# SCoulY/MuSCLe

Hardware: AMD Instinct MI355X
Metric: images/sec (whole node), MCL EfficientNet-B7 448x448 bs=32/GPU (higher is better)
Workload: dtype f32; 1 GPU; train_mcl.py loop body, step-A (epoch-4 gates: focal+softmargin+pairwise+ER+IMC, one backward, one Adam step), MuSCLe(efficientnet-b7, last_pooling=False, 21 classes), random-init weights; per_gpu_batch=32, global_batch=32, image=448x448, parallelism=single, optimizer=Adam(lr=1e-4, wd=5e-5) fused, launch=eager, weight-gradient GEMMs on a second stream

## Files before the change

include/muscle_hip.h:

```cpp
#ifndef MUSCLE_HIP_H
#define MUSCLE_HIP_H

#ifdef __cplusplus
extern "C" {
#endif

int mx_version(void);
int mx_abi_hash(void);
const char* mx_last_error(void);


int mx_pw_fwd_parts(int M, int N, int K);
int mx_pw_fwd(const float* A, int a_mode, const float* a_scale, const float* a_shift, const float* a_gate,
              int rows_per_sample, const float* W, float* C, int M, int K, int N, int lda, int ldc,
              const float* bias, const float* residual, int relu, float* stats, void* stream);

int mx_set_gemm_mode(int mode);
int mx_get_gemm_mode(void);
int mx_set_wgrad_kernel(int kernel, int groups);
int mx_get_wgrad_kernel(void);
int mx_gemm_uses_split(int kind, int M, int N, int K);

long mx_pw_planes_bytes(int N, int K);
int mx_pw_planes_tiles(int N, int K);
int mx_pw_planes_batch(const long* table, int n, int total_tiles, void* stream);
int mx_pw_fwd_uses_planes(int M, int K, int N);
int mx_pw_fwd_planes(const float* A, const void* Wplanes, float* C, int M, int K, int N, int lda, int ldc,
                     const float* bias, const float* residual, int relu, float* stats, void* stream);

int mx_transpose(const float* src, float* dst, int rows, int cols, void* stream);
int mx_transpose_batch(const long* table, int n, int total_tiles, void* stream);

int mx_pw_dgrad(const float* G, const float* W, float* dX, int M, int K, int N, int ldg, int ldx,
                const float* residual, void* stream);

int mx_pw_dgrad_bnbwd(const float* G, const float* X, const float* coef, const float* Wt, float* dX, float* dZ, int M, int K, int N,
                      int ldg, int ldx, const float* residual, void* stream);

int mx_pw_fwd_act_uses_planes(int M, int K, int N);
int mx_pw_fwd_planes_act(const float* A, const float* scale, const float* shift, const float* gate, int rows_per_sample,
                         const void* Wplanes, float* C, int M, int K, int N, int lda, int ldc, float* stats, void* stream);

int mx_pw_dgrad_bnbwd_planes(const float* G, const float* X, const float* coef, const void* WtPlanes, float* dX, int M, int K, int N,
                             int ldg, int ldx, const float* residual, void* stream);
int mx_pw_wgrad_tile_bnbwd_ok(int R, int Co, int Ci);
int mx_pw_wgrad_small_bnbwd_ok(int R, int Co, int Ci);
int mx_pw_wgrad_small_bnbwd(const float* G, const float* G2, const float* coef, const float* X, float* dW, int R, int Co, int Ci,
                            int ldg, int ldx, void* ws, long ws_bytes, void* stream);
int mx_pw_wgrad_tile_bnbwd(const float* G, const float* G2, const float* coef, const float* X, float* dW, int R, int Co, int Ci,
                           int ldg, int ldx, void* ws, long ws_bytes, void* stream);
int mx_pw_wgrad_tile_bnbwd_dz_ok(int R, int Co, int Ci, int ldg, int ldx);
int mx_pw_wgrad_tile_bnbwd_dz(const float* G, const float* G2, const float* coef, const float* X, float* dW, float* dz, int R, int Co,
                              int Ci, int ldg, int ldx, void* ws, long ws_bytes, void* stream);

long mx_pw_wgrad_ws(int R, int Co, int Ci);
int mx_pw_wgrad(const float* G, const float* X, int x_mode, const float* x_scale, const float* x_shift,
                const float* x_gate, int rows_per_sample, float* dW, int R, int Co, int Ci, int ldg, int ldx,
                void* ws, long ws_bytes, void* stream);

long mx_pw_wgrad_small_ws(int R, int Co, int Ci, int x_mode);
int mx_pw_wgrad_small(const float* G, const float* X, int x_mode, const float* x_scale, const float* x_shift,
                      const float* x_gate, int rows_per_sample, float* dW, int R, int Co, int Ci, int ldg, int ldx,
                      void* ws, long ws_bytes, void* stream);

int mx_pw_bwd_small_fused_ok(int R, int Co, int Ci);
int mx_pw_bwd_small_fused_groups(int R, int Co, int Ci);
int mx_pw_bwd_small_fused(const float* G, const float* G2, const float* coef, const float* X, const float* W, float* dW, float* dX,
                          const float* residual, int R, int Co, int Ci, int ldg, int ldx, int lddx, void* ws, long ws_bytes, void* stream);
int mx_pw_parts_reduce(const float* part, int groups, int n, float* dW, void* stream);

int mx_pw_proj_bwd_fused_ok(int R, int Cout, int Cexp, int rows_per_sample);
int mx_pw_proj_bwd_fused_groups(int R, int Cout, int Cexp, int rows_per_sample);
int mx_pw_proj_bwd_fused(const float* dp, const float* d_raw, const float* scale, const float* shift, const float* gate, int rows_per_sample,
                         const float* Wp, float* dW, float* dA, float* out5, int R, int Cout, int Cexp, int lddp, int ldraw, int ldda,
                         void* ws, long ws_bytes, void* stream);

long mx_pw_wgrad_tile_ws(int R, int Co, int Ci, int x_mode);
int mx_pw_wgrad_tile(const float* G, const float* X, int x_mode, const float* x_scale, const float* x_shift,
                     const float* x_gate, int rows_per_sample, float* dW, int R, int Co, int Ci, int ldg, int ldx,
                     void* ws, long ws_bytes, void* stream);

int mx_bgemm(int layout, const float* A, const float* B, float* C, int M, int N, int K, int lda, int ldb, int ldc,
             long sa, long sb, long sc, int batch, int relu, void* stream);


int mx_colreduce_parts(long rows, int C);
int mx_colstats(const float* X, long rows, int C, float* part, void* stream);

int mx_bn_finalize(const float* part, int P, int C, double count, const float* gamma, const float* beta, float* running_mean,
                   float* running_var, float momentum, float eps, int training, float* scale, float* shift,
                   float* mean, float* rstd, double* acc , void* stream);

int mx_fold_block(const float* We, const float* g0, const float* b0, const float* m0, const float* v0, float eps0,
                  const float* g1, const float* b1, const float* m1, const float* v1, float eps1,
                  const float* Wp, const float* g2, const float* b2, const float* m2, const float* v2, float eps2,
                  int Cin, int Cexp, int Cout, float* We_f, float* be, float* s1, float* t1, float* Wp_f, float* bp, void* stream);

int mx_bn_apply(const float* P, const float* scale, const float* shift, const float* row_scale, const float* residual,
                const float* gate, float* out, long rows, int C, int rows_per_sample, int act, void* stream);

int mx_bn_bwd_reduce(const float* G, const float* X, const float* row_scale, const float* gate, const float* gate_add,
                     const float* act_scale, const float* act_shift, long rows, int C, int rows_per_sample,
                     float* part, void* stream);

int mx_bn_bwd_finalize(const float* part, int P, int C, double count, const float* gamma, const float* mean, const float* rstd,
                       int training, float* dgamma, float* dbeta, float* c1, float* c2, float* c3, double* acc,
                       void* stream);

int mx_bn_bwd_apply(const float* G, const float* X, const float* row_scale, const float* gate, const float* gate_add,
                    const float* act_scale, const float* act_shift, const float* c1, const float* c2, const float* c3,
                    float* out, long rows, int C, int rows_per_sample, void* stream);

long mx_pool_ws(long rows, int C, int rows_per_sample, int planes);
int mx_pool_sum(const float* X, const float* G, const float* scale, const float* shift, int act, long rows, int C,
                int rows_per_sample, float* out, void* ws, long ws_bytes, void* stream);

int mx_se_bn1_pool(const float* dA, const float* X, const float* scale, const float* shift, long rows, int C, int rows_per_sample,
                   float* out5, void* ws, long ws_bytes, void* stream);
int mx_bn1_sums_finalize(const float* pooled5, const float* gate, const float* gh, const float* W1, float inv_hw, float* add,
                         int N, int C, int SQ, double count, const float* gamma, const float* mean, const float* rstd, int training,
                         float* dgamma, float* dbeta, float* c1, float* c2, float* c3, void* stream);


int mx_dwconv_fwd_parts(int N, int Ho, int Wo, int C, int S);
long mx_dwconv_fwd_ws(int N, int Ho, int Wo, int C, int S);
int mx_dwconv_fwd(const float* X, const float* scale, const float* shift, const float* W, float* Y, float* stats,
                  const float* pool_scale, const float* pool_shift, float* pooled, void* ws, long ws_bytes, int N,
                  int H, int Wd, int C, int K, int S, int pad_lo, int Ho, int Wo, void* stream);

int mx_dwconv_bwd_data(const float* dY, const float* W, const float* residual, float* dX, int N, int H, int Wd, int C,
                       int K, int S, int pad_lo, int Ho, int Wo, void* stream);

int mx_dwconv_bwd_weight_parts(int N, int Ho, int Wo, int C, int S);
int mx_dwconv_bwd_weight(const float* X, const float* scale, const float* shift, const float* dY, float* dW, float* dw_scratch,
                         int N, int H, int Wd, int C, int K, int S, int pad_lo, int Ho, int Wo, void* stream);

int mx_dwconv_bwd_fused_parts(int N, int H, int Wd, int C, int K);
int mx_dwconv_bwd_fused(const float* dA, const float* D, const float* gate, const float* add, const float* a1, const float* b1,
                        const float* c1, const float* c2, const float* c3, const float* X, const float* a0, const float* b0,
                        const float* W, const float* residual, float* gX, float* dW, float* dw_scratch, float* part, int N, int H,
                        int Wd, int C, int K, int pad_lo, void* stream);

int mx_dwconv_bwd_fused_bn0(const float* dA, const float* D, const float* gate, const float* add, const float* a1, const float* b1,
                            const float* c1, const float* c2, const float* c3, const float* X, const float* a0, const float* b0,
                            const float* W, float* gX, float* dW, float* dw_scratch, float* part, int N, int H, int Wd, int C, int K,
                            int pad_lo, void* ws, long ws_bytes, double count, const float* gamma, const float* mean, const float* rstd,
                            int training, float* dgamma, float* dbeta, float* o1, float* o2, float* o3, void* stream);

int mx_dwconv_bwd_fused_s2_parts(int N, int H, int Wd, int C, int K);
int mx_dwconv_bwd_fused_s2(const float* dA, const float* D, const float* gate, const float* add, const float* a1, const float* b1,
                           const float* c1, const float* c2, const float* c3, const float* X, const float* a0, const float* b0,
                           const float* W, float* gX, float* dW, float* dw_scratch, float* part, int N, int H, int Wd, int C, int K,
                           int pad_lo, int Ho, int Wo, void* stream);

int mx_dw_parts_reduce(const float* part, int P, int n, float* dW, void* stream);


int mx_se_fwd(const float* pooled_sum, float inv_hw, const float* W1, const float* b1, const float* W2, const float* b2,
// ... 233 lines not shown
```

muscle_amd/engine.py:

```python
from __future__ import annotations

import os

from dataclasses import dataclass, field
from typing import Dict, List, Optional

import torch

from . import ops
from .arch import BlockCfg, NetCfg
from .ops import BNState


@dataclass
class BlockTape:
    cfg: BlockCfg
    H: int
    W: int
    Ho: int
    Wo: int
    x: torch.Tensor
    x_st: Optional[BNState]
    e_raw: Optional[torch.Tensor] = None
    bn0: Optional[BNState] = None
# ... 205 lines not shown
            t.x = None
            tape.blocks.append(t)
            if b.index == 0:
                tape.cols = tape.stem_raw = None
            if len(tape.blocks) >= 2 and tape.blocks[-2].cfg.index not in cfg.taps:
                tape.blocks[-2].out = None
            x, x_st, h, w = t.out, None, ho, wo
            continue
        M, Mo = N * h * w, N * ho * wo
        if b.expand:
            assert x_st is None
            st0 = None
            t.e_raw = ops.pw_fwd(x.view(M, b.cin), m._expand_conv.weight.view(b.cexp, b.cin), b.cexp, want_stats=training,
                                 planes=tape.wp.get(id(m._expand_conv.weight)))
            if training:
                t.e_raw, st0 = t.e_raw
            t.e_raw = t.e_raw.view(N, h, w, b.cexp)
            t.bn0 = ops.bn_finalize(st0, M, m._bn0, training)
            dw_in, dw_st = t.e_raw, t.bn0
        else:
            dw_in, dw_st = x, x_st
        st1 = None
        t.d_raw = ops.dwconv_fwd(dw_in, m._depthwise_conv.weight, b.kernel, b.stride, b.pad_lo, ho, wo, st=dw_st,
                                 want_stats=training)
        if training:
            t.d_raw, st1 = t.d_raw
        t.bn1 = ops.bn_finalize(st1, Mo, m._bn1, training)
        d2 = t.d_raw.view(Mo, b.cexp)
        pooled = ops.pool_sum(d2, ho * wo, st=t.bn1, act=True)
        t.s, t.h, t.gate = ops.se_fwd(pooled, 1.0 / (ho * wo), m._se_reduce.weight.view(b.se, b.cexp), m._se_reduce.bias,
                                      m._se_expand.weight.view(b.cexp, b.se), m._se_expand.bias)
        st2 = None
        if b.cout > MATERIALISE_ABOVE:
            t.a = ops.bn_apply(d2, t.bn1, gate=t.gate, rows_per_sample=ho * wo, act=True)
            t.p_raw = ops.pw_fwd(t.a, m._project_conv.weight.view(b.cout, b.cexp), b.cout, want_stats=training,
                                 planes=tape.wp.get(id(m._project_conv.weight)))
        else:
            t.p_raw = ops.pw_fwd(d2, m._project_conv.weight.view(b.cout, b.cexp), b.cout, a_mode=ops.BNACT,
                                 a_scale=t.bn1.scale, a_shift=t.bn1.shift, a_gate=t.gate, rows_per_sample=ho * wo,
                                 want_stats=training, planes=tape.wp.get(id(m._project_conv.weight)))
        if training:
            t.p_raw, st2 = t.p_raw
        t.bn2 = ops.bn_finalize(st2, Mo, m._bn2, training)
        if b.skip and training and b.drop_rate:
            if drop_u is not None:
                keep = 1.0 - b.drop_rate
                t.row_scale = torch.floor(keep + drop_u[b.index].to(dev, torch.float32)) / keep
            else:
                t.row_scale = drop_scales[b.index]
        res = None
        if b.skip:
            assert x_st is None
            res = x.view(M, b.cin)
        t.out = ops.bn_apply(t.p_raw, t.bn2, row_scale=t.row_scale, residual=res, rows_per_sample=ho * wo).view(N, ho, wo, b.cout)
        tape.blocks.append(t)
        x, x_st, h, w = t.out, None, ho, wo
        if not save:
            t.x = t.e_raw = t.d_raw = t.p_raw = t.a = None
            if b.index == 0:
                tape.cols = tape.stem_raw = None
            if len(tape.blocks) >= 2 and tape.blocks[-2].cfg.index not in cfg.taps:
                tape.blocks[-2].out = None
    ops.flush_batch_counters()
    return tape


class GradSink:

    def __init__(self):
        self.bufs: Dict[int, torch.Tensor] = {}

    def of(self, p: torch.nn.Parameter) -> torch.Tensor:
        g = self.bufs.get(id(p))
        if g is None:
            g = torch.zeros_like(p, memory_format=torch.contiguous_format)
            self.bufs[id(p)] = g
        return g


FOLD_BN0_EARLY = os.environ.get("MUSCLE_FOLD_BN0_EARLY", "1") == "1"
DW_S2_FUSED = os.environ.get("MUSCLE_DW_S2_FUSED", "1") == "1"
PW_BWD_FUSED = os.environ.get("MUSCLE_PW_BWD_FUSED", "1") == "1"
PW_PROJ_BWD_FUSED = os.environ.get("MUSCLE_PW_PROJ_BWD_FUSED", "1") == "1"
WGRAD_SIDE_STREAM = os.environ.get("MUSCLE_WGRAD_STREAM", "1") == "1"
_side_streams: Dict[int, "torch.cuda.Stream"] = {}


class _WgradLane:
    def __init__(self, device):
        self.s = None
        self.pending = []
        self.keep = []
        if WGRAD_SIDE_STREAM:
            key = device.index if device.index is not None else torch.cuda.current_device()
            if key not in _side_streams:
                _side_streams[key] = torch.cuda.Stream(device=device)
            self.s = _side_streams[key]

    def _queue(self, launch, *reads):
        if self.s is None:
            return launch()
        self.pending.append((launch, reads))

    def wgrad(self, G, X, dW, **kw):
        return self._queue(lambda: ops.pw_wgrad(G, X, dW, **kw), G, X)

    def wgrad_bnbwd(self, G, G2, coef, X, dW):
        return self._queue(lambda: ops.pw_wgrad_bnbwd(G, G2, coef, X, dW), G, X, G2, coef)

    def dw_reduce(self, scratch, dW):
        return self._queue(lambda: ops.dw_parts_reduce(scratch, dW), scratch)

    def pw_reduce(self, part, dW):
        return self._queue(lambda: ops.pw_parts_reduce(part, dW), part)

    def flush(self):
        if self.s is None or not self.pending:
            return
        self.s.wait_stream(torch.cuda.current_stream())
        with torch.cuda.stream(self.s):
            for launch, _ in self.pending:
                launch()
        self.keep.extend(reads for _, reads in self.pending)
        self.pending = []

    def progress(self, done, module):
        if self.s is None:
            return done(module)
        self.flush()
        self.s.wait_stream(torch.cuda.current_stream())
        with torch.cuda.stream(self.s):
            done(module)

    def join(self):
        self.flush()
        if self.s is not None:
            torch.cuda.current_stream().wait_stream(self.s)
        self.keep = []


def _dw_input(t: BlockTape):
    return (t.e_raw, t.bn0) if t.cfg.expand else (t.x, t.x_st)


def _project_backward(lane, tape: Tape, t: BlockTape, m, g_out, sink: GradSink):
    b, hw = t.cfg, t.Ho * t.Wo
    Mo = tape.N * hw
    dp = ops.bn_backward(g_out.reshape(Mo, b.cout), t.p_raw, m._bn2, t.bn2, sink.of(m._bn2.weight), sink.of(m._bn2.bias), tape.training,
                         row_scale=t.row_scale, rows_per_sample=hw)
    if t.a is None and PW_PROJ_BWD_FUSED:
        takes = getattr(ops, "pw_proj_bwd_fused_takes", None)
        if takes is not None and takes(Mo, b.cout, b.cexp, hw):
            ga, pooled5 = ops.pw_proj_bwd_fused(dp, t.d_raw.view(Mo, b.cexp), t.bn1, t.gate, hw, m._project_conv.weight.view(b.cout, b.cexp),
                                                sink.of(m._project_conv.weight).view(b.cout, b.cexp), defer=lane.pw_reduce)
            lane.flush()
            return ga, pooled5
    if t.a is not None:
        lane.wgrad(dp, t.a, sink.of(m._project_conv.weight).view(b.cout, b.cexp))
        t.a = None
    else:
        lane.wgrad(dp, t.d_raw.view(Mo, b.cexp), sink.of(m._project_conv.weight).view(b.cout, b.cexp), x_mode=ops.BNACT,
                   x_scale=t.bn1.scale, x_shift=t.bn1.shift, x_gate=t.gate, rows_per_sample=hw)
    ga = ops.pw_dgrad(dp, m._project_conv.weight.view(b.cout, b.cexp), b.cexp, wt=tape.wt.get(id(m._project_conv.weight)),
                      planes=tape.wtp.get(id(m._project_conv.weight)))
    lane.flush()
    return ga, None


def _se_bn1_coeffs(tape: Tape, t: BlockTape, m, ga, pooled5, sink: GradSink):
    b, hw = t.cfg, t.Ho * t.Wo
    Mo = tape.N * hw
    if pooled5 is None:
        pooled5 = ops.se_bn1_pool(ga, t.d_raw.view(Mo, b.cexp), t.bn1, hw)
    gh = ops.se_bwd(pooled5[0], t.gate, t.s, t.h, m._se_expand.weight.view(b.cexp, b.se),
                    sink.of(m._se_reduce.weight).view(b.se, b.cexp), sink.of(m._se_reduce.bias),
                    sink.of(m._se_expand.weight).view(b.cexp, b.se), sink.of(m._se_expand.bias))
    return ops.bn1_coeffs(pooled5, t.gate, gh, m._se_reduce.weight.view(b.se, b.cexp), 1.0 / hw, Mo, m._bn1, t.bn1,
                          sink.of(m._bn1.weight), sink.of(m._bn1.bias), tape.training)


def _depthwise_backward(lane, tape: Tape, t: BlockTape, m, ga, c1, add, skip_res, sink: GradSink):
    b, N = t.cfg, tape.N
    dw_in, dw_st = _dw_input(t)
    res = None if dw_st is not None else skip_res
    if b.stride == 1 and b.pad_lo == (b.kernel - 1) // 2:
        return ops.dwconv_bwd_fused(ga.view(N, t.Ho, t.Wo, b.cexp), t.d_raw, t.gate, add, t.bn1, c1, dw_in, dw_st,
                                    m._depthwise_conv.weight, sink.of(m._depthwise_conv.weight), b.kernel, b.pad_lo,
                                    residual=res, defer=lane.dw_reduce)
    if DW_S2_FUSED and b.stride == 2 and dw_st is not None:
        return ops.dwconv_bwd_fused_s2(ga.view(N, t.Ho, t.Wo, b.cexp), t.d_raw, t.gate, add, t.bn1, c1, dw_in, dw_st,
                                       m._depthwise_conv.weight, sink.of(m._depthwise_conv.weight), b.kernel, b.pad_lo,
                                       defer=lane.dw_reduce)
    dd = ops.bn_backward_from_coeffs(ga, t.d_raw.view(N * t.Ho * t.Wo, b.cexp), t.bn1, c1, gate=t.gate, gate_add=add,
                                     rows_per_sample=t.Ho * t.Wo, out=ga).view(N, t.Ho, t.Wo, b.cexp)
    ops.dwconv_bwd_weight(dw_in, dd, sink.of(m._depthwise_conv.weight), b.kernel, b.stride, b.pad_lo, st=dw_st)
    return ops.dwconv_bwd_data(dd, m._depthwise_conv.weight, b.kernel, b.stride, b.pad_lo, t.H, t.W, residual=res), None


def _bn0_expand_backward(lane, backbone, cfg: NetCfg, tape: Tape, t: BlockTape, m, gx, part0, skip_res, sink: GradSink):
    b, N, training = t.cfg, tape.N, tape.training
    dw_in, dw_st = _dw_input(t)
    bn_mod = m._bn0 if b.expand else backbone._bn0
    M = N * t.H * t.W
    raw2, gx2 = dw_in.view(M, dw_in.shape[3]), gx.view(M, dw_in.shape[3])
    res = skip_res.reshape(M, b.cin) if skip_res is not None else None
    if part0 is not None:
        c0 = ops.bn_bwd_coeffs(part0, M, bn_mod, dw_st, sink.of(bn_mod.weight), sink.of(bn_mod.bias), training)
        wtp = tape.wtp.get(id(m._expand_conv.weight)) if b.expand else None
        takes = None
        if FOLD_BN0_EARLY and b.expand and (wtp is not None if b.stride == 1 else PW_BWD_FUSED):
            takes = ops.bnbwd_fold_takes(M, b.cexp, b.cin)
            if takes == "fused" and not PW_BWD_FUSED:
                takes = ops.bnbwd_fold_takes_split(M, b.cexp, b.cin)
        if takes == "fused":
            g_in = ops.pw_bwd_fused(gx2, raw2, c0, t.x.view(M, b.cin), m._expand_conv.weight.view(b.cexp, b.cin),
                                    sink.of(m._expand_conv.weight).view(b.cexp, b.cin), residual=res, defer=lane.pw_reduce)
            lane.flush()
            return g_in.view(N, t.H, t.W, b.cin)
        if takes == "small" and b.stride == 1:
            lane.wgrad_bnbwd(gx2, raw2, c0, t.x.view(M, b.cin), sink.of(m._expand_conv.weight).view(b.cexp, b.cin))
            g_in = ops.pw_dgrad_bnbwd_planes(gx2, raw2, c0, wtp, b.cin, residual=res)
            lane.flush()
            return g_in.view(N, t.H, t.W, b.cin)
        dz = ops.bn_bwd_apply_plain(gx2, raw2, c0, gx2)
    else:
        dz = ops.bn_backward(gx2, raw2, bn_mod, dw_st, sink.of(bn_mod.weight), sink.of(bn_mod.bias), training, act=dw_st, out=gx2)
    if not b.expand:
        dw28 = torch.zeros(cfg.stem_out, 28, dtype=torch.float32, device=dz.device)
        ops.pw_wgrad(dz, tape.cols, dw28)
        sink.of(backbone._conv_stem.weight).view(cfg.stem_out, 27).add_(dw28[:, :27])
# ... 34 lines not shown
```

muscle_amd/ops.py:

```python
from __future__ import annotations

import os
from typing import NamedTuple, Optional

import torch

from ._lib import call, lib, ptr, stream

PLAIN, BNACT, AFFINE = 0, 1, 2


class BNState(NamedTuple):
    scale: torch.Tensor
    shift: torch.Tensor
    mean: torch.Tensor
    rstd: torch.Tensor


def _f32(*shape, device):
    return torch.empty(shape, dtype=torch.float32, device=device)


_scratch_bufs: dict = {}
_wgrad_ws: dict = {}
# ... 224 lines not shown
    if lib().mx_pw_wgrad_small_bnbwd_ok(M, K, N):
        return "small"
    if lib().mx_pw_wgrad_small_ws(M, K, N, PLAIN) <= 0 and lib().mx_pw_wgrad_tile_bnbwd_ok(M, K, N):
        return "tile"
    return None


def pw_wgrad_bnbwd(G, G2, coef, X, dW):
    R, Co = G.shape
    Ci = X.shape[1]
    if lib().mx_pw_wgrad_small_bnbwd_ok(R, Co, Ci):
        need = lib().mx_pw_wgrad_small_ws(R, Co, Ci, PLAIN)
        ws = _wgrad_workspace(G.device, max(need, 16))
        call("mx_pw_wgrad_small_bnbwd", ptr(G), ptr(G2), ptr(coef), ptr(X), ptr(dW), R, Co, Ci, G.stride(0), X.stride(0), ws.data_ptr(), ws.numel(), stream())
        return
    need = lib().mx_pw_wgrad_tile_ws(R, Co, Ci, PLAIN)
    ws = _wgrad_workspace(G.device, max(need, 16))
    call("mx_pw_wgrad_tile_bnbwd", ptr(G), ptr(G2), ptr(coef), ptr(X), ptr(dW), R, Co, Ci, G.stride(0), X.stride(0), ws.data_ptr(), ws.numel(), stream())


def _rows_ptr(t, what):
    if t is None:
        return None
    if not t.is_cuda or t.dtype != torch.float32 or t.dim() != 2 or t.stride(1) != 1:
        raise ValueError(f"{what} must be a 2-D fp32 CUDA tensor with unit column stride")
    return t.data_ptr()


def pw_parts_reduce(part, dW):
    P, n = part.shape
    call("mx_pw_parts_reduce", ptr(part), P, n, ptr(dW), stream())


def pw_bwd_fused(G, G2, coef, X, W, dW, *, residual=None, defer=None, out=None):
    R, Co = G.shape
    Ci = X.shape[1]
    dX = out if out is not None else _f32(R, Ci, device=G.device)
    if G2 is not None and G2.stride(0) != G.stride(0):
        raise ValueError("pw_bwd_fused: G2 must share G's leading dimension")
    if residual is not None and residual.stride(0) != dX.stride(0):
        raise ValueError("pw_bwd_fused: residual must share dX's leading dimension")
    groups = lib().mx_pw_bwd_small_fused_groups(R, Co, Ci)
    if defer is not None and groups > 0:
        part = _f32(groups, Co * Ci, device=G.device)
        wsp, wsn, dwp = part.data_ptr(), part.numel() * 4, None
    else:
        part = None
        ws = _wgrad_workspace(G.device, max(lib().mx_pw_wgrad_small_ws(R, Co, Ci, PLAIN), 16))
        wsp, wsn, dwp = ws.data_ptr(), ws.numel(), ptr(dW)
    call("mx_pw_bwd_small_fused", _rows_ptr(G, "G"), _rows_ptr(G2, "G2"), ptr(coef), _rows_ptr(X, "X"), ptr(W), dwp, _rows_ptr(dX, "dX"),
         _rows_ptr(residual, "residual"), R, Co, Ci, G.stride(0), X.stride(0), dX.stride(0), wsp, wsn, stream())
    if part is not None:
        defer(part, dW)
    return dX


def pw_proj_bwd_fused_takes(R, Cout, Cexp, rows_per_sample) -> bool:
    return bool(lib().mx_pw_proj_bwd_fused_ok(R, Cout, Cexp, rows_per_sample))


def pw_proj_bwd_fused(dp, d_raw2d, st1: "BNState", gate, rows_per_sample, Wp, dW, *, defer=None, out=None):
    R, Cout = dp.shape
    Cexp = d_raw2d.shape[1]
    groups = lib().mx_pw_proj_bwd_fused_groups(R, Cout, Cexp, rows_per_sample)
    if groups <= 0:
        raise ValueError(f"pw_proj_bwd_fused: R={R} Cout={Cout} Cexp={Cexp} rows_per_sample={rows_per_sample} not taken")
    N = R // rows_per_sample
    dA = out if out is not None else _f32(R, Cexp, device=dp.device)
    pooled5 = _f32(5, N, Cexp, device=dp.device)
    n_part, n_pool = groups * Cout * Cexp, (groups + N - 1) * 5 * Cexp
    if defer is not None:
        ws = _f32(n_part + n_pool, device=dp.device)
        wsp, wsn, dwp = ws.data_ptr(), ws.numel() * 4, None
    else:
        ws = _wgrad_workspace(dp.device, (n_part + n_pool) * 4)
        wsp, wsn, dwp = ws.data_ptr(), ws.numel(), ptr(dW)
    call("mx_pw_proj_bwd_fused", _rows_ptr(dp, "dp"), _rows_ptr(d_raw2d, "d_raw"), ptr(st1.scale), ptr(st1.shift), ptr(gate), rows_per_sample,
         ptr(Wp), dwp, _rows_ptr(dA, "dA"), ptr(pooled5), R, Cout, Cexp, dp.stride(0), d_raw2d.stride(0), dA.stride(0), wsp, wsn, stream())
    if defer is not None:
        defer(ws[:n_part].view(groups, Cout * Cexp), dW)
    return dA, pooled5


def wgrad_bnbwd_dz_takes(R, Co, Ci) -> bool:
    return bool(lib().mx_pw_wgrad_tile_bnbwd_dz_ok(R, Co, Ci, Co, Ci))


def pw_wgrad_bnbwd_dz(G, G2, coef, X, dW, dz=None):
    R, Co = G.shape
    Ci = X.shape[1]
    if dz is None:
        dz = torch.empty_like(G)
    need = lib().mx_pw_wgrad_tile_ws(R, Co, Ci, PLAIN)
    ws = _wgrad_workspace(G.device, max(need, 16))
    call("mx_pw_wgrad_tile_bnbwd_dz", ptr(G), ptr(G2), ptr(coef), ptr(X), ptr(dW), ptr(dz), R, Co, Ci, G.stride(0), X.stride(0),
         ws.data_ptr(), ws.numel(), stream())
    return dz


WGRAD_TILE = os.environ.get("MUSCLE_WGRAD_TILE", "1") == "1"
WGRAD_SMALL = True


def pw_wgrad(G, X, dW, *, x_mode=PLAIN, x_scale=None, x_shift=None, x_gate=None, rows_per_sample=1):
    R, Co = G.shape
    Ci = X.shape[1]
    if WGRAD_SMALL and dW.is_contiguous():
        need = lib().mx_pw_wgrad_small_ws(R, Co, Ci, x_mode)
        if need > 0:
            ws = _wgrad_workspace(G.device, need)
            call("mx_pw_wgrad_small", ptr(G), ptr(X), x_mode, ptr(x_scale), ptr(x_shift), ptr(x_gate), rows_per_sample, ptr(dW),
                 R, Co, Ci, G.stride(0), X.stride(0), ws.data_ptr(), ws.numel(), stream())
            return
    if WGRAD_TILE and dW.is_contiguous():
        need = lib().mx_pw_wgrad_tile_ws(R, Co, Ci, x_mode)
        if need > 0:
            ws = _wgrad_workspace(G.device, need)
            call("mx_pw_wgrad_tile", ptr(G), ptr(X), x_mode, ptr(x_scale), ptr(x_shift), ptr(x_gate), rows_per_sample, ptr(dW),
                 R, Co, Ci, G.stride(0), X.stride(0), ws.data_ptr(), ws.numel(), stream())
            return
    need = lib().mx_pw_wgrad_ws(R, Co, Ci)
    ws = _wgrad_workspace(G.device, need) if need > 0 else None
    call("mx_pw_wgrad", ptr(G), ptr(X), x_mode, ptr(x_scale), ptr(x_shift), ptr(x_gate), rows_per_sample, ptr(dW),
         R, Co, Ci, G.stride(0), X.stride(0), ws.data_ptr() if ws is not None else None, ws.numel() if ws is not None else 0, stream())


def bgemm(layout, A, B, out, M, N, K, *, relu=False):
    b = A.shape[0]
    call("mx_bgemm", layout, ptr(A), ptr(B), ptr(out), M, N, K, A.stride(1), B.stride(1), out.stride(1),
         A.stride(0), B.stride(0), out.stride(0), b, int(relu), stream())
    return out


def colstats(X2d):
    rows, C = X2d.shape
    part = _f32(lib().mx_colreduce_parts(rows, C), 2, C, device=X2d.device)
    call("mx_colstats", ptr(X2d), rows, C, ptr(part), stream())
    return part


def bn_finalize(stats, count, bn: torch.nn.BatchNorm2d, training: bool) -> BNState:
    C = bn.num_features
    dev = bn.weight.device
    buf = _f32(4, C, device=dev)
    b0, b1, b2, b3 = buf.unbind(0)
    base = buf.data_ptr()
    mom = 0.0 if bn.momentum is None else float(bn.momentum)
    call("mx_bn_finalize", ptr(stats), stats.shape[0] if stats is not None else 0, C, float(count), ptr(bn.weight), ptr(bn.bias), ptr(bn.running_mean),
         ptr(bn.running_var), mom, float(bn.eps), int(training), base, base + 4 * C, base + 8 * C, base + 12 * C,
         _acc_scratch(dev, 128 * C) if training else None, stream())
    if training:
        _nbt_pending.append(bn.num_batches_tracked)
    return BNState(b0, b1, b2, b3)


def fold_block(We, bn0, bn1, Wp, bn2, out=None):
    dev = Wp.device
    cout, cexp = Wp.shape
    cin = We.shape[1] if We is not None else cexp
    if out is not None:
        f, vec = out, out["_vec"]
    else:
        f = {}
        vec = f["_vec"] = _f32(3, cexp, device=dev)
        if We is not None:
            f["We"], f["be"] = _f32(cexp, cin, device=dev), vec[0]
        f["bn1"] = BNState(vec[1], vec[2], None, None)
        f["Wp"], f["bp"] = _f32(cout, cexp, device=dev), _f32(cout, device=dev)

    def four(bn):
        return (ptr(bn.weight), ptr(bn.bias), ptr(bn.running_mean), ptr(bn.running_var), float(bn.eps))
    none4 = (None, None, None, None, 0.0)
    call("mx_fold_block", ptr(We.detach()) if We is not None else None, *(four(bn0) if We is not None else none4), *four(bn1),
         ptr(Wp.detach()), *four(bn2), cin, cexp, cout, ptr(f.get("We")), ptr(f.get("be")), ptr(vec[1]), ptr(vec[2]),
         ptr(f["Wp"]), ptr(f["bp"]), stream())
    return f


_nbt_pending: list = []


def flush_batch_counters():
    if _nbt_pending:
        torch._foreach_add_(_nbt_pending, 1)
        _nbt_pending.clear()


def bn_apply(P2d, st: BNState, *, row_scale=None, residual=None, gate=None, rows_per_sample=1, act=False, out=None):
    rows, C = P2d.shape
    if out is None:
        out = torch.empty_like(P2d)
    call("mx_bn_apply", ptr(P2d), ptr(st.scale), ptr(st.shift), ptr(row_scale), ptr(residual), ptr(gate), ptr(out), rows, C,
         rows_per_sample, int(act), stream())
    return out


def bn_backward(G2d, X2d, bn: torch.nn.BatchNorm2d, st: BNState, dgamma, dbeta, training: bool, *, row_scale=None,
                gate=None, gate_add=None, act: Optional[BNState] = None, rows_per_sample=1, out=None):
    rows, C = X2d.shape
    P = lib().mx_colreduce_parts(rows, C)
    sums = _f32(P, 2, C, device=X2d.device)
    a_sc = act.scale if act is not None else None
    a_sh = act.shift if act is not None else None
    call("mx_bn_bwd_reduce", ptr(G2d), ptr(X2d), ptr(row_scale), ptr(gate), ptr(gate_add), ptr(a_sc), ptr(a_sh), rows, C,
         rows_per_sample, ptr(sums), stream())
    c = _f32(3, C, device=X2d.device)
    call("mx_bn_bwd_finalize", ptr(sums), P, C, float(rows), ptr(bn.weight), ptr(st.mean), ptr(st.rstd), int(training),
         ptr(dgamma), ptr(dbeta), ptr(c[0]), ptr(c[1]), ptr(c[2]),
         _acc_scratch(X2d.device, 128 * C), stream())
    if out is None:
        out = torch.empty_like(X2d)
    call("mx_bn_bwd_apply", ptr(G2d), ptr(X2d), ptr(row_scale), ptr(gate), ptr(gate_add), ptr(a_sc), ptr(a_sh),
         ptr(c[0]), ptr(c[1]), ptr(c[2]), ptr(out), rows, C, rows_per_sample, stream())
    return out


def bn_backward_from_coeffs(G2d, X2d, st: BNState, c, *, gate, gate_add, rows_per_sample, out):
    rows, C = X2d.shape
    cb, cs = c.data_ptr(), 4 * C
    call("mx_bn_bwd_apply", ptr(G2d), ptr(X2d), None, ptr(gate), ptr(gate_add), ptr(st.scale), ptr(st.shift),
         cb, cb + cs, cb + 2 * cs, ptr(out), rows, C, rows_per_sample, stream())
    return out


def bn_bwd_coeffs(part, rows, bn, st: BNState, dgamma, dbeta, training: bool):
    P, _, C = part.shape
    c = _f32(3, C, device=part.device)
    base = c.data_ptr()
    call("mx_bn_bwd_finalize", ptr(part), P, C, float(rows), ptr(bn.weight), ptr(st.mean), ptr(st.rstd), int(training),
         ptr(dgamma), ptr(dbeta), base, base + 4 * C, base + 8 * C, _acc_scratch(part.device, 128 * C), stream())
    return c


def bn_bwd_apply_plain(G2d, X2d, c, out):
    rows, C = X2d.shape
    cb, cs = c.data_ptr(), 4 * c.shape[1]
    call("mx_bn_bwd_apply", ptr(G2d), ptr(X2d), None, None, None, None, None, cb, cb + cs, cb + 2 * cs, ptr(out),
         rows, C, 1, stream())
    return out


def dw_parts_reduce(scratch, dW):
    P, n = scratch.shape
    call("mx_dw_parts_reduce", ptr(scratch), P, n, ptr(dW), stream())


def dwconv_bwd_fused(dA, D, gate, add, st1: BNState, c1, X, st0: Optional[BNState], W, dW, K, pad_lo, *, residual=None, defer=None,
                     bn0=None):
    N, H, Wd, C = X.shape
    gX = _f32(N, H, Wd, C, device=X.device)
    P = lib().mx_dwconv_bwd_fused_parts(N, H, Wd, C, K)
    part = _f32(P, 2, C, device=X.device) if st0 is not None else None
    scratch = _f32(P, C * K * K, device=X.device)
    cb, cs = c1.data_ptr(), 4 * c1.shape[1]
    if bn0 is not None and st0 is not None and residual is None:
        bn, dgamma, dbeta, training = bn0
        co = _f32(3, C, device=X.device)
        ob = co.data_ptr()
        ws, wsn = _scratch(X.device, 65536)
        _call_ws("mx_dwconv_bwd_fused_bn0", ptr(dA), ptr(D), ptr(gate), ptr(add), ptr(st1.scale), ptr(st1.shift), cb, cb + cs, cb + 2 * cs,
                 ptr(X), ptr(st0.scale), ptr(st0.shift), ptr(W), ptr(gX), None if defer is not None else ptr(dW), ptr(scratch), ptr(part),
                 N, H, Wd, C, K, pad_lo, ws, wsn, float(N * H * Wd), ptr(bn.weight), ptr(st0.mean), ptr(st0.rstd), int(training),
                 ptr(dgamma), ptr(dbeta), ob, ob + 4 * C, ob + 8 * C, stream())
        if defer is not None:
            defer(scratch, dW)
        return gX, part, co
    call("mx_dwconv_bwd_fused", ptr(dA), ptr(D), ptr(gate), ptr(add), ptr(st1.scale), ptr(st1.shift), cb, cb + cs,
         cb + 2 * cs, ptr(X), ptr(st0.scale) if st0 else None, ptr(st0.shift) if st0 else None, ptr(W), ptr(residual), ptr(gX),
         None if defer is not None else ptr(dW), ptr(scratch), ptr(part), N, H, Wd, C, K, pad_lo, stream())
    if defer is not None:
        defer(scratch, dW)
    return (gX, part, None) if bn0 is not None else (gX, part)


def dwconv_bwd_fused_s2(dA, D, gate, add, st1: BNState, c1, X, st0: BNState, W, dW, K, pad_lo, *, defer=None):
    N, H, Wd, C = X.shape
    _, Ho, Wo, _ = D.shape
    gX = _f32(N, H, Wd, C, device=X.device)
    P = lib().mx_dwconv_bwd_fused_s2_parts(N, H, Wd, C, K)
    part = _f32(P, 2, C, device=X.device)
    scratch = _f32(P, C * K * K, device=X.device)
    cb, cs = c1.data_ptr(), 4 * c1.shape[1]
    call("mx_dwconv_bwd_fused_s2", ptr(dA), ptr(D), ptr(gate), ptr(add), ptr(st1.scale), ptr(st1.shift), cb, cb + cs, cb + 2 * cs,
         ptr(X), ptr(st0.scale), ptr(st0.shift), ptr(W), ptr(gX), None if defer is not None else ptr(dW), ptr(scratch), ptr(part),
         N, H, Wd, C, K, pad_lo, Ho, Wo, stream())
    if defer is not None:
        defer(scratch, dW)
    return gX, part


def se_bn1_pool(dA2d, X2d, st: BNState, rows_per_sample):
    rows, C = X2d.shape
    N = rows // rows_per_sample
    out = _f32(5, N, C, device=X2d.device)
    ws, wsn = _scratch(X2d.device, lib().mx_pool_ws(rows, C, rows_per_sample, 5))
    _call_ws("mx_se_bn1_pool", ptr(dA2d), ptr(X2d), ptr(st.scale), ptr(st.shift), rows, C, rows_per_sample, ptr(out), ws, wsn, stream())
    return out
# ... 280 lines not shown
```

Before: 348.5 images/sec.

## Fuse BN backward apply into streaming projection-conv backward kernel

Adds a streaming HIP kernel that recomputes the BN2 backward output from the reduce coefficients inside the projection-conv backward, doing dgrad, wgrad and SE pooling partial sums in one pass with MFMA. This avoids materialising dp through a separate bn_bwd_apply kernel and then re-reading it. It applies only to Cout=32 with Cexp 32/64 and very large row counts, and adds a per-sample pooling reduction kernel plus a new workspace layout.

```diff
diff --git a/include/muscle_hip.h b/include/muscle_hip.h
--- a/include/muscle_hip.h
+++ b/include/muscle_hip.h
@@ -74,6 +74,13 @@
 int mx_pw_proj_bwd_fused(const float* dp, const float* d_raw, const float* scale, const float* shift, const float* gate, int rows_per_sample,
                          const float* Wp, float* dW, float* dA, float* out5, int R, int Cout, int Cexp, int lddp, int ldraw, int ldda,
                          void* ws, long ws_bytes, void* stream);
+
+int mx_pw_proj_bwd_stream_ok(int R, int Cout, int Cexp, int rows_per_sample);
+int mx_pw_proj_bwd_stream_groups(int R, int Cout, int Cexp, int rows_per_sample);
+int mx_pw_proj_bwd_stream(const float* g, const float* p_raw, const float* coef, const float* row_scale, const float* d_raw,
+                          const float* scale, const float* shift, const float* gate, int rows_per_sample, const float* Wp, float* dW,
+                          float* dA, float* out5, int R, int Cout, int Cexp, int ldg, int ldp, int ldraw, int ldda, void* ws, long ws_bytes,
+                          void* stream);
 
 long mx_pw_wgrad_tile_ws(int R, int Co, int Ci, int x_mode);
 int mx_pw_wgrad_tile(const float* G, const float* X, int x_mode, const float* x_scale, const float* x_shift,
diff --git a/muscle_amd/csrc/wgrad_proj_stream.hip b/muscle_amd/csrc/wgrad_proj_stream.hip
--- /dev/null
+++ b/muscle_amd/csrc/wgrad_proj_stream.hip
@@ -0,0 +1,309 @@
+#include "common.h"
+
+typedef float f32x4s __attribute__((ext_vector_type(4)));
+typedef float f32x2s __attribute__((ext_vector_type(2)));
+
+struct WsArgs {
+  const float* G;
+  const float* P;
+  const float* coef;
+  const float* rs;
+  const float* X;
+  const float* ca;
+  const float* cb;
+  const float* gate;
+  const float* W;
+  float* part;
+  float* dA;
+  float* pp;
+  int R, ldg, ldp, ldx, ldda, rps, rows_per_wave;
+};
+
+static __device__ __forceinline__ __amdgpu_buffer_rsrc_t ws_rsrc(const float* base, long bytes) {
+  const unsigned long long p = (unsigned long long)base;
+  const unsigned lo = __builtin_amdgcn_readfirstlane((unsigned)p), hi = __builtin_amdgcn_readfirstlane((unsigned)(p >> 32));
+  const unsigned n = __builtin_amdgcn_readfirstlane((unsigned)bytes);
+  return __builtin_amdgcn_make_buffer_rsrc((void*)(((unsigned long long)hi << 32) | lo), 0, n, 0x00020000);
+}
+
+template <int V> struct WsVec;
+template <> struct WsVec<2> {
+  typedef f32x2s T;
+  static __device__ __forceinline__ T load(__amdgpu_buffer_rsrc_t r, unsigned vo, unsigned so) {
+    return __builtin_bit_cast(T, __builtin_amdgcn_raw_buffer_load_b64(r, vo, so, 0));
+  }
+  static __device__ __forceinline__ void store(T v, __amdgpu_buffer_rsrc_t r, unsigned vo, unsigned so) {
+    __builtin_amdgcn_raw_buffer_store_b64(__builtin_bit_cast(decltype(__builtin_amdgcn_raw_buffer_load_b64(r, 0, 0, 0)), v), r, vo, so, 0);
+  }
+};
+template <> struct WsVec<4> {
+  typedef f32x4s T;
+  static __device__ __forceinline__ T load(__amdgpu_buffer_rsrc_t r, unsigned vo, unsigned so) {
+    return __builtin_bit_cast(T, __builtin_amdgcn_raw_buffer_load_b128(r, vo, so, 0));
+  }
+  static __device__ __forceinline__ void store(T v, __amdgpu_buffer_rsrc_t r, unsigned vo, unsigned so) {
+    __builtin_amdgcn_sched_barrier(0);
+    __builtin_amdgcn_raw_buffer_store_b128(__builtin_bit_cast(decltype(__builtin_amdgcn_raw_buffer_load_b128(r, 0, 0, 0)), v), r, vo, so, 0);
+    asm volatile("s_nop 3" ::: "memory");
+    __builtin_amdgcn_sched_barrier(0);
+  }
+};
+
+constexpr int WS_CO = 32, WS_SG = 48, WS_TW = 16 * WS_SG;
+constexpr long ws_lds_floats(int CI) {
+  const long work = 4L * WS_TW + 8L * 64 * (CI / 16) + 96, join = 4L * WS_CO * CI;
+  return work > join ? work : join;
+}
+
+template <int CI, bool FOLD>
+__global__ __launch_bounds__(256, CI == 32 ? 4 : 2) void pw_proj_stream_kernel(WsArgs a) {
+  extern __shared__ __attribute__((aligned(16))) float smem[];
+  constexpr int CO = WS_CO, TCI = CI / 16, SG = WS_SG, RB = 16;
+  typedef WsVec<TCI> XV;
+  typedef typename XV::T xvec;
+  const int tid = threadIdx.x, lane = tid & 63, wave = __builtin_amdgcn_readfirstlane(tid >> 6);
+  const int l15 = lane & 15, q = lane >> 4;
+  float* const T = smem + wave * WS_TW;
+  float* const wl = smem + 4 * WS_TW;
+  float* const cf = wl + 8 * 64 * TCI;
+
+#pragma unroll
+  for (int t = wave; t < 8; t += 4) {
+    const int K = 16 * (t >> 2) + 4 * q + (t & 3);
+    *reinterpret_cast<xvec*>(wl + (t * 64 + lane) * TCI) = *reinterpret_cast<const xvec*>(a.W + K * CI + TCI * l15);
+  }
+  if (FOLD && tid < 96) cf[tid] = a.coef[tid];
+  __syncthreads();
+
+  const long gw = (long)blockIdx.x * 4 + wave;
+  const long w_end = min((long)a.R, (gw + 1) * a.rows_per_wave);
+  const int rows = (int)max(0L, w_end - gw * a.rows_per_wave);
+  const long w_beg = rows > 0 ? gw * a.rows_per_wave : 0;
+  const int ns = rows / RB;
+  const __amdgpu_buffer_rsrc_t rsg = ws_rsrc(a.G + w_beg * a.ldg, rows > 0 ? ((long)(rows - 1) * a.ldg + CO) * 4 : 0);
+  const __amdgpu_buffer_rsrc_t rsp = ws_rsrc(FOLD ? a.P + w_beg * a.ldp : a.G, FOLD && rows > 0 ? ((long)(rows - 1) * a.ldp + CO) * 4 : 0);
+  const __amdgpu_buffer_rsrc_t rsx = ws_rsrc(a.X + w_beg * a.ldx, rows > 0 ? ((long)(rows - 1) * a.ldx + CI) * 4 : 0);
+  const __amdgpu_buffer_rsrc_t rsa = ws_rsrc(a.dA + w_beg * a.ldda, rows > 0 ? ((long)(rows - 1) * a.ldda + CI) * 4 : 0);
+  const int prow = 4 * (l15 & 3) + (l15 >> 2);
+  const unsigned vog = (unsigned)(prow * a.ldg + 4 * q) * 4u, vop = (unsigned)(prow * a.ldp + 4 * q) * 4u;
+  const unsigned vox = (unsigned)(q * a.ldx + TCI * l15) * 4u, voa = (unsigned)(q * a.ldda + TCI * l15) * 4u;
+
+  const xvec ca = *reinterpret_cast<const xvec*>(a.ca + TCI * l15), cb = *reinterpret_cast<const xvec*>(a.cb + TCI * l15);
+
+  f32x4s acc[2][TCI];
+#pragma unroll
+  for (int i = 0; i < 2; ++i)
+#pragma unroll
+    for (int n = 0; n < TCI; ++n) acc[i][n] = f32x4s{0.f, 0.f, 0.f, 0.f};
+
+  f32x4s gN[2], pN[2];
+  xvec xN[4];
+#define WS_LOAD_X(S, D) XV::load(rsx, vox, (unsigned)(((S) * RB + 4 * (D)) * a.ldx) * 4u)
+#define WS_ISSUE_GP(S)                                                                                                   \
+  _Pragma("unroll") for (int e_ = 0; e_ < 2; ++e_) {                                                                     \
+    gN[e_] = WsVec<4>::load(rsg, vog + 64u * e_, (unsigned)((S) * RB * a.ldg) * 4u);                                     \
+    if (FOLD) pN[e_] = WsVec<4>::load(rsp, vop + 64u * e_, (unsigned)((S) * RB * a.ldp) * 4u);                           \
+  }
+  float sum[5][TCI];
+#pragma unroll
+  for (int n = 0; n < TCI; ++n)
+#pragma unroll
+    for (int i = 0; i < 5; ++i) sum[i][n] = 0.f;
+  int smp = 0, s_end = 0;
+  xvec cg = ca;
+  float rsv = 1.f;
+  if (ns > 0) {
+    WS_ISSUE_GP(0)
+#pragma unroll
+    for (int d = 0; d < 4; ++d) xN[d] = WS_LOAD_X(0, d);
+    smp = (int)((unsigned long)w_beg / (unsigned)a.rps);
+    s_end = (int)min((long)ns, ((long)(smp + 1) * a.rps - w_beg) / RB);
+    cg = *reinterpret_cast<const xvec*>(a.gate + (long)smp * CI + TCI * l15);
+    if (FOLD && a.rs) rsv = a.rs[smp];
+  }
+  for (int s = 0; s < ns; ++s) {
+    const int sn = min(s + 1, ns - 1);
+    f32x4s dp[2];
+    xvec x[4];
+#pragma unroll
+    for (int e = 0; e < 2; ++e) {
+      if (FOLD) {
+        const f32x4s k1 = *reinterpret_cast<const f32x4s*>(cf + 16 * e + 4 * q), k2 = *reinterpret_cast<const f32x4s*>(cf + 32 + 16 * e + 4 * q),
+                     k3 = *reinterpret_cast<const f32x4s*>(cf + 64 + 16 * e + 4 * q);
+#pragma unroll
+        for (int j = 0; j < 4; ++j) dp[e][j] = k1[j] * (gN[e][j] * rsv) + k2[j] * pN[e][j] + k3[j];
+      } else {
+        dp[e] = gN[e];
+      }
+    }
+    WS_ISSUE_GP(sn)
+#pragma unroll
+    for (int d = 0; d < 4; ++d) { x[d] = xN[d]; xN[d] = WS_LOAD_X(sn, d); }
+#pragma unroll
+    for (int e = 0; e < 2; ++e) *reinterpret_cast<f32x4s*>(T + prow * SG + 16 * e + 4 * q) = dp[e];
+    f32x4s da[TCI];
+#pragma unroll
+    for (int n = 0; n < TCI; ++n) da[n] = f32x4s{0.f, 0.f, 0.f, 0.f};
+#pragma unroll
+    for (int t = 0; t < 8; ++t) {
+      const xvec w = *reinterpret_cast<const xvec*>(wl + (t * 64 + lane) * TCI);
+#pragma unroll
+      for (int n = 0; n < TCI; ++n) da[n] = __builtin_amdgcn_mfma_f32_16x16x4f32(dp[t >> 2][t & 3], w[n], da[n], 0, 0, 0);
+    }
+#pragma unroll
+    for (int r = 0; r < 4; ++r) {
+      xvec o;
+#pragma unroll
+      for (int n = 0; n < TCI; ++n) o[n] = da[n][r];
+      XV::store(o, rsa, voa, (unsigned)((s * RB + 4 * r) * a.ldda) * 4u);
+    }
+    __builtin_amdgcn_fence(__ATOMIC_RELEASE, "wavefront");
+    __builtin_amdgcn_wave_barrier();
+    __builtin_amdgcn_fence(__ATOMIC_ACQUIRE, "wavefront");
+#pragma unroll
+    for (int d = 0; d < 4; ++d) {
+      const float g0 = T[(4 * d + q) * SG + l15], g1 = T[(4 * d + q) * SG + 16 + l15];
+#pragma unroll
+      for (int n = 0; n < TCI; ++n) {
+        const float xv = x[d][n];
+        const float z = ca[n] * xv + cb[n];
+        const float sg = sigmoidf_(z);
+        const float act = z * sg;
+        const float bv = act * cg[n];
+        const float sp = sg * (1.f + z * (1.f - sg)), dv = da[n][d];
+        sum[0][n] += dv * act; sum[1][n] += dv * sp; sum[2][n] += sp;
+        sum[3][n] += dv * sp * xv; sum[4][n] += sp * xv;
+        acc[0][n] = __builtin_amdgcn_mfma_f32_16x16x4f32(g0, bv, acc[0][n], 0, 0, 0);
+        acc[1][n] = __builtin_amdgcn_mfma_f32_16x16x4f32(g1, bv, acc[1][n], 0, 0, 0);
+      }
+    }
+    __builtin_amdgcn_fence(__ATOMIC_RELEASE, "wavefront");
+    __builtin_amdgcn_wave_barrier();
+    if (s + 1 == s_end) {
+      float* dst = a.pp + (gw + smp) * 5 * CI + TCI * l15;
+#pragma unroll
+      for (int n = 0; n < TCI; ++n)
+#pragma unroll
+        for (int i = 0; i < 5; ++i) {
+          float v = sum[i][n];
+          v += __shfl_xor(v, 16, 64);
+          v += __shfl_xor(v, 32, 64);
+          if (q == 0) dst[i * CI + n] = v;
+          sum[i][n] = 0.f;
+        }
+      if (s + 1 < ns) {
+        ++smp;
+        s_end = (int)min((long)ns, ((long)(smp + 1) * a.rps - w_beg) / RB);
+        cg = *reinterpret_cast<const xvec*>(a.gate + (long)smp * CI + TCI * l15);
+            if (FOLD && a.rs) rsv = a.rs[smp];
+      }
+    }
+  }
+#undef WS_ISSUE_GP
+#undef WS_LOAD_X
+
+  __syncthreads();
+  float* const J = smem + wave * CO * CI;
+#pragma unroll
+  for (int i = 0; i < 2; ++i)
+#pragma unroll
+    for (int n = 0; n < TCI; ++n)
+#pragma unroll
+      for (int r = 0; r < 4; ++r) J[(16 * i + 4 * q + r) * CI + TCI * l15 + n] = acc[i][n][r];
+  __syncthreads();
+  float* out = a.part + (long)blockIdx.x * CO * CI;
+#pragma unroll
+  for (int e = tid; e < CO * CI; e += 256) out[e] = ((smem[e] + smem[CO * CI + e]) + smem[2 * CO * CI + e]) + smem[3 * CO * CI + e];
+}
+
+__global__ __launch_bounds__(256) void pw_proj_stream_pool_kernel(const float* __restrict__ pp, int rps, int rows_per_wave, int Ci, int N,
+                                                                  float* __restrict__ out5) {
+  __shared__ double sh[16][17];
+  const int el = threadIdx.x & 15, k = threadIdx.x >> 4, e = blockIdx.x * 16 + el, n = blockIdx.y;
+  const int g0 = (int)((long)n * rps / rows_per_wave), g1 = (int)(((long)(n + 1) * rps - 1) / rows_per_wave);
+  const int per = (g1 - g0 + 16) / 16, ga = g0 + k * per, gb = min(g1 + 1, ga + per);
+  double s = 0.0;
+  if (e < 5 * Ci)
+    for (int g = ga; g < gb; ++g) s += (double)pp[(long)(g + n) * 5 * Ci + e];
+  sh[k][el] = s;
+  __syncthreads();
+  if (k == 0 && e < 5 * Ci) {
+#pragma unroll
+    for (int j = 1; j < 16; ++j) s += sh[j][el];
+    const int i = e / Ci, c = e - i * Ci;
+    out5[((long)i * N + n) * Ci + c] = (float)s;
+  }
+}
+
+static bool wps_shape(int Co, int Ci) { return Co == 32 && (Ci == 32 || Ci == 64); }
+
+struct WpsPlan { int rows_per_wave, waves, groups; };
+static bool wps_plan(int R, int Co, int Ci, int rps, WpsPlan* p) {
+  if (R < 16 || rps < 16 || rps % 16 || R % rps || R / rps > 65535 || !wps_shape(Co, Ci)) return false;
+  const int round_waves = 256 * 4 * (Ci == 32 ? 4 : 2);
+  int rows = cdiv(cdiv(R, round_waves), 16) * 16;
+  if (rows < 32) rows = 32;
+  p->rows_per_wave = rows;
+  p->waves = cdiv(R, rows);
+  p->groups = cdiv(p->waves, 4);
+  return true;
+}
+
+template <int CI, bool FOLD>
+static void wps_launch(const WsArgs& a, const WpsPlan& p, hipStream_t st) {
+  hipLaunchKernelGGL((pw_proj_stream_kernel<CI, FOLD>), dim3(p.groups), dim3(256), ws_lds_floats(CI) * 4, st, a);
+}
+
+extern "C" {
+
+int mx_pw_proj_bwd_stream_ok(int R, int Cout, int Cexp, int rows_per_sample) {
+  WpsPlan p;
+  return R >= 65536 && wps_plan(R, Cout, Cexp, rows_per_sample, &p) ? 1 : 0;
+}
+
+int mx_pw_proj_bwd_stream_groups(int R, int Cout, int Cexp, int rows_per_sample) {
+  WpsPlan p;
+  return wps_plan(R, Cout, Cexp, rows_per_sample, &p) ? p.groups : 0;
+}
+
+int mx_pw_proj_bwd_stream(const float* g, const float* p_raw, const float* coef, const float* row_scale, const float* d_raw,
+                          const float* scale, const float* shift, const float* gate, int rows_per_sample, const float* Wp, float* dW,
+                          float* dA, float* out5, int R, int Cout, int Cexp, int ldg, int ldp, int ldraw, int ldda, void* ws, long ws_bytes,
+                          void* stream) {
+  MX_CHECK_ARG(wps_shape(Cout, Cexp) && R >= 16, "pw_proj_bwd_stream: shape R=%d Cout=%d Cexp=%d not taken (32 x 32 and 32 x 64 only)", R, Cout, Cexp);
+  MX_CHECK_ARG(rows_per_sample >= 16 && rows_per_sample % 16 == 0 && R % rows_per_sample == 0,
+               "pw_proj_bwd_stream: rows_per_sample=%d must be a multiple of 16 that divides R=%d", rows_per_sample, R);
+  MX_CHECK_ARG(g && d_raw && scale && shift && gate && Wp && dA && out5 && ws, "pw_proj_bwd_stream: null pointer");
+  MX_CHECK_ARG((p_raw != nullptr) == (coef != nullptr), "pw_proj_bwd_stream: p_raw and coef come together (both null: g is dp)");
+  MX_CHECK_ARG(p_raw || !row_scale, "pw_proj_bwd_stream: row_scale belongs to the folded form");
+  MX_CHECK_ARG((((uintptr_t)g | (uintptr_t)p_raw | (uintptr_t)coef | (uintptr_t)d_raw | (uintptr_t)scale | (uintptr_t)shift | (uintptr_t)gate |
+                 (uintptr_t)Wp | (uintptr_t)dW | (uintptr_t)dA | (uintptr_t)out5 | (uintptr_t)ws) & 15) == 0 && ((uintptr_t)row_scale & 3) == 0,
+               "pw_proj_bwd_stream: pointers must be 16-byte aligned");
+  MX_CHECK_ARG(ldg % 4 == 0 && ldraw % 4 == 0 && ldda % 4 == 0 && ldg >= Cout && ldraw >= Cexp && ldda >= Cexp && (!p_raw || (ldp % 4 == 0 && ldp >= Cout)),
+               "pw_proj_bwd_stream: leading dimensions (%d, %d, %d, %d) must be multiples of 4 and cover the rows", ldg, ldp, ldraw, ldda);
+  WpsPlan p;
+  MX_CHECK_ARG(wps_plan(R, Cout, Cexp, rows_per_sample, &p), "pw_proj_bwd_stream: no plan for R=%d Cout=%d Cexp=%d", R, Cout, Cexp);
+  const long ldmax = std::max(std::max((long)ldg, (long)(p_raw ? ldp : 0)), std::max((long)ldraw, (long)ldda));
+  MX_CHECK_ARG((long)p.rows_per_wave * ldmax * 4 < (1L << 31), "pw_proj_bwd_stream: a wave's rows must span less than 2 GB (leading dimension %ld)", ldmax);
+  const int N = R / rows_per_sample;
+  const long part_floats = (long)p.groups * Cout * Cexp;
+  MX_CHECK_ARG(ws_bytes >= (part_floats + (long)(4L * p.groups + N - 1) * 5 * Cexp) * 4, "pw_proj_bwd_stream: workspace too small");
+  WsArgs a{};
+  a.G = g; a.P = p_raw; a.coef = coef; a.rs = row_scale; a.X = d_raw; a.ca = scale; a.cb = shift; a.gate = gate; a.W = Wp;
+  a.part = (float*)ws; a.dA = dA; a.pp = (float*)ws + part_floats;
+  a.R = R; a.ldg = ldg; a.ldp = p_raw ? ldp : ldg; a.ldx = ldraw; a.ldda = ldda; a.rps = rows_per_sample; a.rows_per_wave = p.rows_per_wave;
+  hipStream_t st = (hipStream_t)stream;
+  if (Cexp == 32) { if (p_raw) wps_launch<32, true>(a, p, st); else wps_launch<32, false>(a, p, st); }
+  else { if (p_raw) wps_launch<64, true>(a, p, st); else wps_launch<64, false>(a, p, st); }
+  MX_LAUNCH_CHECK();
+  hipLaunchKernelGGL(pw_proj_stream_pool_kernel, dim3(cdiv(5 * Cexp, 16), N), dim3(256), 0, st, (const float*)a.pp, rows_per_sample,
+                     p.rows_per_wave, Cexp, N, out5);
+  MX_LAUNCH_CHECK();
+  if (dW) {
+    mx_launch_parts_reduce((const float*)ws, p.groups, Cout * Cexp, dW, st);
+    MX_LAUNCH_CHECK();
+  }
+  return MX_OK;
+}
+
+}
diff --git a/muscle_amd/engine.py b/muscle_amd/engine.py
--- a/muscle_amd/engine.py
+++ b/muscle_amd/engine.py
@@ -311,6 +311,7 @@
 DW_S2_FUSED = os.environ.get("MUSCLE_DW_S2_FUSED", "1") == "1"
 PW_BWD_FUSED = os.environ.get("MUSCLE_PW_BWD_FUSED", "1") == "1"
 PW_PROJ_BWD_FUSED = os.environ.get("MUSCLE_PW_PROJ_BWD_FUSED", "1") == "1"
+PW_PROJ_BWD_STREAM = os.environ.get("MUSCLE_PW_PROJ_BWD_STREAM", "1") == "1"
 WGRAD_SIDE_STREAM = os.environ.get("MUSCLE_WGRAD_STREAM", "1") == "1"
 _side_streams: Dict[int, "torch.cuda.Stream"] = {}
 
@@ -375,6 +376,17 @@
 def _project_backward(lane, tape: Tape, t: BlockTape, m, g_out, sink: GradSink):
     b, hw = t.cfg, t.Ho * t.Wo
     Mo = tape.N * hw
+    if t.a is None and PW_PROJ_BWD_STREAM:
+        takes = getattr(ops, "pw_proj_bwd_stream_takes", None)
+        if takes is not None and takes(Mo, b.cout, b.cexp, hw):
+            g2d = g_out.reshape(Mo, b.cout)
+            coef = ops.bn_backward_coeffs(g2d, t.p_raw, m._bn2, t.bn2, sink.of(m._bn2.weight), sink.of(m._bn2.bias), tape.training,
+                                          row_scale=t.row_scale, rows_per_sample=hw)
+            ga, pooled5 = ops.pw_proj_bwd_stream(g2d, t.p_raw, coef, t.row_scale, t.d_raw.view(Mo, b.cexp), t.bn1, t.gate, hw,
+                                                 m._project_conv.weight.view(b.cout, b.cexp),
+                                                 sink.of(m._project_conv.weight).view(b.cout, b.cexp), defer=lane.pw_reduce)
+            lane.flush()
+            return ga, pooled5
     dp = ops.bn_backward(g_out.reshape(Mo, b.cout), t.p_raw, m._bn2, t.bn2, sink.of(m._bn2.weight), sink.of(m._bn2.bias), tape.training,
                          row_scale=t.row_scale, rows_per_sample=hw)
     if t.a is None and PW_PROJ_BWD_FUSED:
diff --git a/muscle_amd/ops.py b/muscle_amd/ops.py
--- a/muscle_amd/ops.py
+++ b/muscle_amd/ops.py
@@ -330,6 +330,38 @@
     return dA, pooled5
 
 
+def pw_proj_bwd_stream_takes(R, Cout, Cexp, rows_per_sample) -> bool:
+    return bool(lib().mx_pw_proj_bwd_stream_ok(R, Cout, Cexp, rows_per_sample))
+
+
+def pw_proj_bwd_stream(g, p_raw, coef, row_scale, d_raw2d, st1: "BNState", gate, rows_per_sample, Wp, dW, *, defer=None, out=None):
+    R, Cout = g.shape
+    Cexp = d_raw2d.shape[1]
+    if (p_raw is None) != (coef is None) or (p_raw is None and row_scale is not None):
+        raise ValueError("pw_proj_bwd_stream: p_raw and coef come together, row_scale only with them")
+    if coef is not None and (tuple(coef.shape) != (3, Cout) or not coef.is_contiguous()):
+        raise ValueError("pw_proj_bwd_stream: coef must be a contiguous [3, Cout] tensor")
+    groups = lib().mx_pw_proj_bwd_stream_groups(R, Cout, Cexp, rows_per_sample)
+    if groups <= 0:
+        raise ValueError(f"pw_proj_bwd_stream: R={R} Cout={Cout} Cexp={Cexp} rows_per_sample={rows_per_sample} not taken")
+    N = R // rows_per_sample
+    dA = out if out is not None else _f32(R, Cexp, device=g.device)
+    pooled5 = _f32(5, N, Cexp, device=g.device)
+    n_part, n_pool = groups * Cout * Cexp, (4 * groups + N - 1) * 5 * Cexp
+    if defer is not None:
+        ws = _f32(n_part + n_pool, device=g.device)
+        wsp, wsn, dwp = ws.data_ptr(), ws.numel() * 4, None
+    else:
+        ws = _wgrad_workspace(g.device, (n_part + n_pool) * 4)
+        wsp, wsn, dwp = ws.data_ptr(), ws.numel(), ptr(dW)
+    call("mx_pw_proj_bwd_stream", _rows_ptr(g, "g"), _rows_ptr(p_raw, "p_raw"), ptr(coef), ptr(row_scale), _rows_ptr(d_raw2d, "d_raw"),
+         ptr(st1.scale), ptr(st1.shift), ptr(gate), rows_per_sample, ptr(Wp), dwp, _rows_ptr(dA, "dA"), ptr(pooled5), R, Cout, Cexp,
+         g.stride(0), p_raw.stride(0) if p_raw is not None else 0, d_raw2d.stride(0), dA.stride(0), wsp, wsn, stream())
+    if defer is not None:
+        defer(ws[:n_part].view(groups, Cout * Cexp), dW)
+    return dA, pooled5
+
+
 def wgrad_bnbwd_dz_takes(R, Co, Ci) -> bool:
     return bool(lib().mx_pw_wgrad_tile_bnbwd_dz_ok(R, Co, Ci, Co, Ci))
 
@@ -461,6 +493,13 @@
     call("mx_bn_bwd_apply", ptr(G2d), ptr(X2d), ptr(row_scale), ptr(gate), ptr(gate_add), ptr(a_sc), ptr(a_sh),
          ptr(c[0]), ptr(c[1]), ptr(c[2]), ptr(out), rows, C, rows_per_sample, stream())
     return out
+
+
+def bn_backward_coeffs(G2d, X2d, bn: torch.nn.BatchNorm2d, st: BNState, dgamma, dbeta, training: bool, *, row_scale=None, rows_per_sample=1):
+    rows, C = X2d.shape
+    sums = _f32(lib().mx_colreduce_parts(rows, C), 2, C, device=X2d.device)
+    call("mx_bn_bwd_reduce", ptr(G2d), ptr(X2d), ptr(row_scale), None, None, None, None, rows, C, rows_per_sample, ptr(sums), stream())
+    return bn_bwd_coeffs(sums, rows, bn, st, dgamma, dbeta, training)
 
 
 def bn_backward_from_coeffs(G2d, X2d, st: BNState, c, *, gate, gate_add, rows_per_sample, out):
```

Result: no change. 351.6 images/sec (median of 6 runs) (+0.9%).
